# enricobottazzi/zk-fhe

Hardware: AMD Instinct MI355X
Metric: BFV proofs/sec (k=13) (higher is better)
Workload: dtype u32x8 (256-bit Montgomery integers over BN254 Fr/Fq)

## Files before the change

### include/zkfhe.h

```cpp
#ifndef ZKFHE_H
#define ZKFHE_H
#include <stddef.h>
#include <stdint.h>

#ifdef __cplusplus
extern "C" {
#endif

#define ZKFHE_OK 0
#define ZKFHE_EINVAL (-1)
#define ZKFHE_EHIP (-2)
#define ZKFHE_ENOMEM (-3)
#define ZKFHE_ENODEV (-4)

typedef struct zkfhe_ctx zkfhe_ctx;
typedef struct zkfhe_basis zkfhe_basis;

typedef struct { uint64_t l[4]; } zkfhe_fr;
typedef struct { uint64_t l[4]; } zkfhe_fq;
typedef struct { zkfhe_fq x, y; } zkfhe_g1_affine;
typedef struct { zkfhe_fq x, y, zz, zzz; } zkfhe_g1_xyzz;

int zkfhe_ctx_create(int device_id, void *hip_stream, zkfhe_ctx **out);
int zkfhe_ctx_destroy(zkfhe_ctx *ctx);
// ... 166 lines not shown
int zkfhe_srs_table_bits(const zkfhe_srs *srs, int *wide_calls);
int zkfhe_srs_table_info(const zkfhe_srs *srs, int bits[2], uint64_t *bytes, int *narrowed);

typedef struct zkfhe_bfv_pk zkfhe_bfv_pk;
int zkfhe_bfv_keygen(zkfhe_ctx *ctx, const zkfhe_srs *srs, const char *input_json, const zkfhe_bfv_params *params,
                     const zkfhe_bfv_config *config, zkfhe_bfv_pk **out);
int zkfhe_bfv_pk_destroy(zkfhe_ctx *ctx, zkfhe_bfv_pk *pk);
int zkfhe_bfv_pk_release_ctx(zkfhe_ctx *ctx, zkfhe_bfv_pk *pk);
int zkfhe_bfv_pk_info(const zkfhe_bfv_pk *pk, uint8_t vk_digest[32], uint32_t *n_fixed, uint32_t *n_sigma);
int zkfhe_bfv_pk_commitments(const zkfhe_bfv_pk *pk, uint8_t *fixed_out, uint8_t *sigma_out);
int zkfhe_bfv_pk_prefix_cache(const zkfhe_bfv_pk *pk, int capacity, uint64_t *hits, uint64_t *misses, uint64_t *entries);
int zkfhe_bfv_pk_prehash(const zkfhe_bfv_pk *pk, const char *input_json, uint64_t *started, uint64_t *taken, uint64_t *pending);
int zkfhe_bfv_pk_break_points(const zkfhe_bfv_pk *pk, int which, uint32_t *out, uint32_t *count);

int zkfhe_bfv_pk_export_vk(const zkfhe_bfv_pk *pk, uint8_t *out, size_t cap, size_t *len);
int zkfhe_bfv_witness_stream(zkfhe_ctx *ctx, const zkfhe_bfv_pk *pk, const char *input_json, const uint8_t gamma_le[32], uint8_t *cells_out,
                             size_t cap_cells, size_t *n_cells);
int zkfhe_lookup_permute(zkfhe_ctx *ctx, const zkfhe_fr *cols_dev, size_t n_cols, size_t n, uint32_t usable_rows, zkfhe_fr *a_dev,
                         zkfhe_fr *s_dev, int *not_in_table);
int zkfhe_bfv_pk_save(zkfhe_ctx *ctx, const zkfhe_bfv_pk *pk, const char *path);
int zkfhe_bfv_pk_load(zkfhe_ctx *ctx, const zkfhe_srs *srs, const char *path, zkfhe_bfv_pk **out);

int zkfhe_snark_encode(const uint8_t *instances_le, size_t n_instances, const uint8_t *proof, size_t proof_len, uint8_t *out, size_t cap, size_t *len);
int zkfhe_snark_decode(const uint8_t *snark, size_t snark_len, uint8_t *instances_le, size_t *n_instances, uint8_t *proof, size_t *proof_len);

int zkfhe_bfv_verify(const uint8_t *vk_bytes, size_t vk_len, const uint8_t *instances, size_t n_instances, const uint8_t *proof,
                     size_t proof_len, const uint8_t *srs_seed, size_t seed_len, int *accepted, char *err, size_t err_len);
int zkfhe_bfv_verify_g2(const uint8_t *vk_bytes, size_t vk_len, const uint8_t *instances, size_t n_instances, const uint8_t *proof, size_t proof_len,
                        const uint8_t g2[128], const uint8_t s_g2[128], int *accepted, char *err, size_t err_len);

// ... 224 lines not shown
```

### zk-fhe_amd/_abi.py

```python
import ctypes
import os

_HERE = os.path.dirname(os.path.abspath(__file__))
LIB_PATH = os.path.join(_HERE, "libzkfhe_hip.so")
_lib = None

PROF_G1_DECOMPRESS, PROF_MSM_SEGMENTED = 3, 4
PROF_BFV_SAMPLE, PROF_RNS_NTT, PROF_RNS_EPILOGUE = 5, 6, 7
PROF_BFV_TENSOR, PROF_BFV_RELIN, PROF_BFV_EVAL_EPILOGUE, PROF_BFV_ELEMENTWISE = 8, 9, 10, 11
PROF_BFV_SHARE_SUM, PROF_BFV_DECRYPT_COMBINE = 12, 13
PROF_BFV_GALOIS, PROF_BFV_SLOT_NTT = 14, 15
PROF_BFV_HOIST, PROF_BFV_LINEAR = 16, 17
PROF_BFV_BSGS_INNER, PROF_BFV_BSGS_GIANT = 18, 19
PROF_BFV_DOT = 20
PROF_BFV_PCKS_COMBINE, PROF_BFV_REFRESH_COMBINE = 21, 22
PROF_G1_FFT = 23
PROF_BFV_BALLOT = 24
PROF_BFV_RESIDENT = 25
PROF_BFV_KEY_SWITCH_WIDE = 26
PROF_BFV_PACK = 27
BALLOT_COUNTED, BALLOT_SKIPPED, BALLOT_BAD_GROUP, BALLOT_NOT_A_CIPHERTEXT, BALLOT_WRONG_KEY, BALLOT_REJECTED, BALLOT_REPEATED = range(7)
BALLOT_STATUSES = 7
BALLOT_STATUS_NAMES = ("counted", "skipped", "bad_group", "not_a_ciphertext", "wrong_key", "rejected", "repeated")
SRS_BAD_POWERS, SRS_BAD_LAGRANGE, SRS_BAD_GENERATOR = 1, 2, 4
# ... 53 lines not shown
    "zkfhe_comm_record_event": "i:vvv", "zkfhe_g1_add": "i:vvvvn", "zkfhe_g1_mul": "i:vvvvn", "zkfhe_g1_fft": "i:vvii",
    "zkfhe_g1_decompress": "i:vvnvv", "zkfhe_msm_segmented": "i:vvnvvnvnv", "zkfhe_witness_poly_mul_u64": "i:vvvnv",
    "zkfhe_host_poly_mul_u32": "i:ppnpp", "zkfhe_witness_div_mod": "i:vvuvvn", "zkfhe_transcript_create": "i:wV", "zkfhe_transcript_destroy": "-:v",
    "zkfhe_transcript_common_scalar": "i:vs", "zkfhe_transcript_write_scalar": "i:vs", "zkfhe_transcript_common_point": "i:vs",
    "zkfhe_transcript_write_point": "i:vs", "zkfhe_transcript_squeeze": "i:vs", "zkfhe_transcript_bytes": "i:vsnN", "zkfhe_poseidon_permute": "i:s",
    "zkfhe_poseidon_constants": "i:ss", "zkfhe_host_hash_mode": "i:i", "zkfhe_poseidon_hash_many": "i:sNnis", "zkfhe_bfv_build_tables": "i:sBCsiVsn",
    "zkfhe_bfv_tables_free": "-:v", "zkfhe_bfv_auto_config": "i:sBwwwWsn", "zkfhe_bfv_tables_count": "n:vi", "zkfhe_bfv_tables_copy_advice": "i:vp",
    "zkfhe_bfv_tables_copy_fixed": "i:vp", "zkfhe_bfv_tables_copy_instance": "i:vp", "zkfhe_bfv_tables_copy_copies": "i:vp",
    "zkfhe_bfv_tables_copy_break_points": "i:viW", "zkfhe_prover_gate": "i:i", "zkfhe_bfv_mock_check": "i:vspsn",
    "zkfhe_bfv_tables_poke_advice": "i:vwws", "zkfhe_srs_create": "i:vwsnV", "zkfhe_srs_save": "i:vvs", "zkfhe_srs_drop_host_copy": "i:v",
    "zkfhe_srs_load": "i:vsV", "zkfhe_srs_g2": "i:vss", "zkfhe_srs_set_g2": "i:vss", "zkfhe_srs_file_g2": "i:sWss", "zkfhe_chacha20_block": "i:sWs",
    "zkfhe_srs_from_points": "i:vwvvV", "zkfhe_srs_from_monomial": "i:vwvnssV", "zkfhe_srs_load_downsized": "i:vswV", "zkfhe_srs_check": "i:vvsW",
    "zkfhe_srs_create_sharded": "i:vvwsnV", "zkfhe_srs_destroy": "i:vv", "zkfhe_srs_table_bits": "i:vI", "zkfhe_srs_table_info": "i:vIpI",
    "zkfhe_bfv_keygen": "i:vvsBCV", "zkfhe_bfv_pk_destroy": "i:vv", "zkfhe_bfv_pk_release_ctx": "i:vv", "zkfhe_bfv_pk_info": "i:vsWW",
    "zkfhe_bfv_pk_commitments": "i:vss", "zkfhe_bfv_pk_prefix_cache": "i:vippp", "zkfhe_bfv_pk_prehash": "i:vsppp",
    "zkfhe_bfv_pk_break_points": "i:viWW", "zkfhe_bfv_pk_export_vk": "i:vsnN", "zkfhe_bfv_witness_stream": "i:vvssvnN",
    "zkfhe_lookup_permute": "i:vvnnwvvI", "zkfhe_bfv_pk_save": "i:vvs", "zkfhe_bfv_pk_load": "i:vvsV", "zkfhe_snark_encode": "i:snsnsnN",
    "zkfhe_snark_decode": "i:snsNsN", "zkfhe_bfv_verify": "i:snsnsnsnIsn", "zkfhe_bfv_verify_g2": "i:snsnsnssIsn",
    "zkfhe_bfv_verify_batch": "i:vsnnSNSNsnssIsn", "zkfhe_bfv_prove": "i:vvvsssnNsNf", "zkfhe_bfv_prove_words": "i:vvvXssnNsNf",
    "zkfhe_poly_mul_ternary_negacyclic": "i:vvnvnuuvI", "zkfhe_bfv_error_cdt": "i:BpN", "zkfhe_bfv_fhe_keypair": "i:vBsppp",
    "zkfhe_bfv_encrypt": "i:vBppnpsuppppp", "zkfhe_bfv_decrypt": "i:vBpnppp", "zkfhe_bfv_add": "i:vBnppppipp", "zkfhe_bfv_sum": "i:vBnpppp",
    "zkfhe_bfv_add_plain": "i:vBnppnppp", "zkfhe_bfv_mul_plain": "i:vBnppnppp", "zkfhe_bfv_relin_digits": "i:BiN",
    "zkfhe_bfv_relin_keygen": "i:vBpsipp", "zkfhe_bfv_mul": "i:vBnppppppipp", "zkfhe_bfv_noise": "i:vBpnppp", "zkfhe_bfv_dot_max_terms": "i:BiN",
    "zkfhe_bfv_dot": "i:vBnnppnppppipp", "zkfhe_bfv_dot_plain": "i:vBnnppnppp", "zkfhe_bfv_keygen_share": "i:vBssppp",
    "zkfhe_bfv_share_aggregate": "i:vBnnpp", "zkfhe_bfv_relin_share1": "i:vBpssipp", "zkfhe_bfv_relin_share2": "i:vBpsippp",
    "zkfhe_bfv_decrypt_share": "i:vBpnpsuup", "zkfhe_bfv_decrypt_combine": "i:vBnnppp", "zkfhe_bfv_pcks_share": "i:vBpppnpsuupp",
    "zkfhe_bfv_pcks_combine": "i:vBnnppppp", "zkfhe_bfv_refresh_share": "i:vBpsnpsuupp", "zkfhe_bfv_refresh_combine": "i:vBnnsuppppp",
    "zkfhe_bfv_slot_count": "i:BN", "zkfhe_bfv_galois_element": "i:Blip", "zkfhe_bfv_slot_sum_elements": "i:BpN", "zkfhe_bfv_encode_slots": "i:vBnpp",
    "zkfhe_bfv_decode_slots": "i:vBnpp", "zkfhe_bfv_galois_keygen": "i:vBpsuipp", "zkfhe_bfv_apply_galois": "i:vBnppuppipp",
    "zkfhe_bfv_slot_sum": "i:vBnppppipp", "zkfhe_bfv_galois_share": "i:vBpssuipp", "zkfhe_bfv_apply_galois_many": "i:vBnppnpppipp",
    "zkfhe_bfv_linear_transform": "i:vBnppnpppippp", "zkfhe_bfv_linear_transform_bsgs": "i:vBnppnpppnpppippp", "zkfhe_bfv_plan_create": "i:vBnpppipV",
# ... 35 lines not shown
```

### zk-fhe_amd/csrc/fr9.hip.hpp

```cpp
#pragma once
#include "lz29.hip.hpp"

namespace zk {

using Fr9S = Lz<0, 1, 1>;
using Fr9C = Lz<0, 1, 32>;
template <int VV>
using Fr9P = Lz<0, 1, (VV <= 160 ? 2 : 3)>;

ZK_HD Fr9S fr9_load(const Fr &w) { return lz_load(w); }
ZK_HD Fr9S fr9_one() { return lz_load(Fr::one()); }
ZK_HD Fr9C fr9_load32(const Fr &w) {
  Fr9C r;
#pragma unroll
  for (int i = 0; i < 9; ++i) {
    const int bit = 29 * i - 5;
    if (i == 0) {
      r.l[0] = (int)((w.l[0] << 5) & q29::MASK);
    } else {
      const int k = bit >> 5, sh = bit & 31;
      u32 v = w.l[k] >> sh;
      if (sh > 3 && k + 1 < 8) v |= w.l[k + 1] << (32 - sh);
      r.l[i] = (int)(v & q29::MASK);
    }
// ... 50 lines not shown
  Fr9S k;
#pragma unroll
  for (int i = 0; i < 9; ++i) k.l[i] = (int)K[i];
  return fr9_mul(c, k);
}

template <int LO, int HI, int V>
ZK_HD Fr fr9_store(const Lz<LO, HI, V> &a) { return lz_store(a); }

ZK_HD Lz<0, 1, 66> fr9_perm_factor(const Fr9C &v, const Lz<0, 1, 2> &t, const Fr9C &gamma) { return fr9_norm(lz_add(lz_add(v, t), gamma)); }
template <int V>
ZK_HD Lz<0, 1, 3> fr9_perm_step(const Lz<0, 1, V> &acc, const Lz<0, 1, 66> &f) { return lz_widen<0, 1, 3>(fr9_mul(acc, f)); }
ZK_HD Lz<0, 1, 2> fr9_lookup_term(const Fr9S &a, const Fr9S &beta, const Lz<0, 1, 64> &s_gamma) { return fr9_mul(lz_add(a, beta), s_gamma); }
ZK_HD Lz<0, 1, 64> fr9_lookup_sum(const Fr9C &s, const Fr9C &gamma) { return fr9_norm(lz_add(s, gamma)); }

}
```

### zk-fhe_amd/host/keygen.hip

```cpp
#include "prover_internal.hpp"

std::vector<BigInt> GpuPolyMul::mul_u64(const std::vector<uint64_t> &a, const std::vector<uint64_t> &b) {
  const U256 *host = mul_u64_raw(a, b);
  std::vector<BigInt> out(2 * a.size() - 1);
  for (size_t i = 0; i < out.size(); ++i) out[i] = fe::to_bigint(host[i]);
  return out;
}

const U256 *GpuPolyMul::mul_u64_raw(const std::vector<uint64_t> &a, const std::vector<uint64_t> &b) {
  const size_t n = a.size();
  if (ws->polyio.bytes < 2 * n * 8 + 2 * n * 32) throw std::runtime_error("polynomial too long for the prover workspace");
  uint64_t *da = (uint64_t *)ws->polyio.p, *db = da + n;
  Fr *dout = (Fr *)(db + n);
  const U256 *host = ws->host_poly;
  int rc = up(ctx, ws, da, a.data(), n * 8);
  if (!rc) rc = up(ctx, ws, db, b.data(), n * 8);
  if (!rc) rc = zkfhe_witness_poly_mul_u64(ctx, da, db, n, (zkfhe_fr *)dout);
  if (!rc) rc = zkfhe_fr_from_mont(ctx, (const zkfhe_fr *)dout, (zkfhe_fr *)dout, 2 * n - 1);
  if (!rc && ws->host_poly && 2 * n - 1 <= ws->host_poly_len) {
    if (zk_memcpy_async(ctx, ws->host_poly, dout, (2 * n - 1) * 32, hipMemcpyDeviceToHost, ctx->stream) != hipSuccess) rc = ZKFHE_EHIP;
    if (!rc) rc = zkfhe_sync(ctx);
  } else if (!rc) {
    pageable.resize(2 * n - 1);
    host = pageable.data();
// ... 25 lines not shown
    std::vector<U256> l(3 * n, fe::zero());
    const size_t u = cfg.u();
    l[0] = fe::one();
    l[n + u] = fe::one();
    for (size_t i = 0; i < u; ++i) l[2 * n + i] = fe::one();
    CK(upload_canon(ctx, ws->key_l_rows(), l.data(), 3 * n));
    CK(extend_cols(ctx, pk, ws, ws->key_l_rows(), 3, pk->l_ext.fr()));
  }
  {
    const Fr wext = zk_fr_root_of_unity((int)cfg.k + 2);
    Fr shift = mont_u64(COSET_G);
    for (int k1 = 0; k1 < pk->ext_rows; ++k1) {
      zkp::k_powers<<<(unsigned)((n + 255) / 256), 256, 0, ctx->stream>>>(shift, dom->omega, pk->xs_ext.fr() + (size_t)k1 * n, n);
      ZK_LAUNCH_CHECK(ctx);
      shift = shift * wext;
    }
    if (pk->ext_rows == 3) {
      CK(pk->ext3_pw.alloc(ctx, 3 * n * 32));
      Fr gk = mont_u64(COSET_G);
      for (int t = 0; t < 3; ++t) {
        zkp::k_powers<<<(unsigned)((n + 255) / 256), 256, 0, ctx->stream>>>(Fr::one(), fr_inv(gk), pk->ext3_pw.fr() + (size_t)t * n, n);
        ZK_LAUNCH_CHECK(ctx);
        gk = gk * wext;
      }
    }
  }
  return ZKFHE_OK;
}

static U256 vk_digest_of(const zkfhe_bfv_pk *pk) { return vk_digest(pk->cfg, pk->fixed_commit, pk->sigma_commit); }
// ... 117 lines not shown
int zkfhe_bfv_keygen(zkfhe_ctx *ctx, const zkfhe_srs *srs, const char *input_json, const zkfhe_bfv_params *params,
                     const zkfhe_bfv_config *config, zkfhe_bfv_pk **out) {
  ZK_ENTER(ctx);
  ZK_ARG(ctx, srs && input_json && params && config && out);
  try {
    return keygen_impl(ctx, srs, input_json, params_from_c(params), config_from_c(config), config->replay != 0, out);
  } catch (const std::exception &e) {
    return zk_fail_msg(ctx, ZKFHE_EINVAL, e.what());
  }
}

int zkfhe_bfv_pk_destroy(zkfhe_ctx *ctx, zkfhe_bfv_pk *pk) {
  ZK_ENTER(ctx);
  if (!pk) return ZKFHE_OK;
  zkfhe_sync(ctx);
  DevBuf *bufs[] = {&pk->fixed_l, &pk->sigma_l, &pk->fixed_ext, &pk->sigma_ext, &pk->l_ext, &pk->xs_ext, &pk->dpow, &pk->ext3_pw,
                    &pk->lookup_src, &pk->inv_slots, &pk->place_start, &pk->place_len};
  for (DevBuf *b : bufs) b->release();
  for (auto &kv : pk->workspaces) free_workspace(kv.second);
  delete pk;
  return ZKFHE_OK;
}

int zkfhe_bfv_pk_release_ctx(zkfhe_ctx *ctx, zkfhe_bfv_pk *pk) {
  ZK_ENTER(ctx);
  ZK_ARG(ctx, pk != nullptr);
  zkfhe_sync(ctx);
  std::lock_guard<std::mutex> lock(pk->mu);
  auto it = pk->workspaces.find(ctx->uid);
  if (it != pk->workspaces.end()) {
    free_workspace(it->second);
// ... 201 lines not shown
}

int zkfhe_bfv_pk_commitments(const zkfhe_bfv_pk *pk, uint8_t *fixed_out, uint8_t *sigma_out) {
  if (!pk) return ZKFHE_EINVAL;
  for (size_t i = 0; i < pk->fixed_commit.size() && fixed_out; ++i) {
    memcpy(fixed_out + 64 * i, pk->fixed_commit[i].x.l, 32);
    memcpy(fixed_out + 64 * i + 32, pk->fixed_commit[i].y.l, 32);
  }
  for (size_t i = 0; i < pk->sigma_commit.size() && sigma_out; ++i) {
    memcpy(sigma_out + 64 * i, pk->sigma_commit[i].x.l, 32);
    memcpy(sigma_out + 64 * i + 32, pk->sigma_commit[i].y.l, 32);
  }
  return ZKFHE_OK;
}

int zkfhe_bfv_pk_export_vk(const zkfhe_bfv_pk *pk, uint8_t *out, size_t cap, size_t *len) {
  if (!pk || !len) return ZKFHE_EINVAL;
  const size_t nf = pk->fixed_commit.size(), ns = pk->sigma_commit.size();
  const size_t need = 8 + 40 + 32 + 64 * (nf + ns);
  *len = need;
  if (!out || cap < need) return out ? ZKFHE_EINVAL : ZKFHE_OK;
  memcpy(out, "ZKFHEVK2", 8);
  const uint32_t hdr[10] = {pk->cfg.k, pk->cfg.n_gate0, pk->cfg.n_gate1, pk->cfg.n_lookup, pk->cfg.n_rlc, pk->cfg.unusable_rows,
                            pk->cfg.lookup_bits, pk->cfg.transcript, (uint32_t)nf, (uint32_t)ns};
  memcpy(out + 8, hdr, 40);
  memcpy(out + 48, pk->vk_digest.l, 32);
  uint8_t *p = out + 80;
  for (const auto &c : pk->fixed_commit) {
    memcpy(p, c.x.l, 32);
    memcpy(p + 32, c.y.l, 32);
// ... 20 lines not shown
```

### zk-fhe_amd/host/prove.hip

```cpp
#include "prover_internal.hpp"

namespace {

void permute_lookup(const std::vector<U256> &input, size_t u, unsigned table_size, std::vector<U256> &a_perm, std::vector<U256> &s_perm) {
  std::vector<size_t> cnt(table_size, 0);
  for (size_t i = 0; i < u; ++i) {
    const U256 &v = input[i];
    if (v.l[1] | v.l[2] | v.l[3] || v.l[0] >= table_size) throw std::runtime_error("lookup input not in table");
    ++cnt[v.l[0]];
  }
  std::vector<size_t> left(table_size, 1);
  left[0] = u - (table_size - 1);
  a_perm.assign(u, fe::zero());
  s_perm.assign(u, fe::zero());
  std::vector<size_t> holes;
  size_t pos = 0;
  for (unsigned v = 0; v < table_size; ++v)
    for (size_t k = 0; k < cnt[v]; ++k, ++pos) {
      a_perm[pos] = fe::from_u64(v);
      if (k == 0) {
        if (!left[v]) throw std::runtime_error("lookup input not in table");
        --left[v];
        s_perm[pos] = fe::from_u64(v);
      } else {
// ... 846 lines not shown
    }
    return ZKFHE_OK;
  }
  zkp::QArgs quotient_args(const zkp::QGroup *groups_dev, int q_rows) const {
    zkp::QArgs qa;
    qa.adv = ws->adv_ext.fr();
    qa.fix = pk->fixed_ext.fr();
    qa.sig = pk->sigma_ext.fr();
    qa.pz = ws->pz_ext.fr();
    qa.lz = ws->lz_ext.fr();
    qa.la = ws->la_ext.fr();
    qa.ls = ws->ls_ext.fr();
    qa.inst = ws->inst_ext.fr();
    qa.lext = pk->l_ext.fr();
    qa.xs = pk->xs_ext.fr();
    qa.beta_delta = beta_delta_dev;
    qa.groups = groups_dev;
    qa.partials = ws->quotient_partials();
    qa.y = y;
    qa.beta = beta;
    qa.gamma = gamma;
    qa.gamma_rlc = mont(gamma_rlc);
    qa.log_n = k;
    qa.u = (unsigned)u;
    qa.n_gate = cfg.n_gate();
    qa.n_rlc = cfg.n_rlc;
    qa.adv_rlc0 = cfg.adv_rlc0();
    qa.fix_qrlc0 = cfg.fix_qrlc0();
    qa.fix_const = cfg.fix_const();
    qa.fix_table = cfg.fix_table();
    qa.adv_lookup0 = cfg.adv_lookup0();
    qa.n_lookup = cfg.n_lookup;
    qa.n_advice = cfg.n_advice();
    qa.n_perm = cfg.n_perm();
    qa.chunk = cfg.chunk();
    qa.n_chunks = cfg.n_chunks();
    qa.rows = (unsigned)q_rows;
    return qa;
  }
  int launch_quotient(zkp::QArgs &qa, size_t pt0, size_t count, size_t G, const Fr *ypow_dev, const Fr *zinv_dev) {
    qa.pt0 = pt0;
    qa.pt_count = count;
    const unsigned blocks = (unsigned)((count + 255) / 256);
    if (G) {
      zkp::k_quotient_partials<<<dim3(blocks, (unsigned)G), 256, 0, ctx->stream>>>(qa);
      ZK_LAUNCH_CHECK(ctx);
    }
    zkp::k_quotient_combine<<<blocks, 256, 0, ctx->stream>>>(ws->quotient_partials(), ypow_dev, (unsigned)G, zinv_dev, k, qa.rows, pt0, count, ws->h_ext.fr());
    ZK_LAUNCH_CHECK(ctx);
    return ZKFHE_OK;
  }
  int quotient(std::vector<AffinePoint> &h_commit) {
    const int q_rows = pk->ext_rows;
    const Fr wext = zk_fr_root_of_unity((int)k + 2);
    if (W_sh == 1) {
      CK(extend_cols(ctx, pk, ws, ws->all_l.fr(), ws->n_all, ws->all_ext.fr()));
    } else {
      const size_t ecol = n * (size_t)q_rows;
      auto ext_range = [&](const View &l, const View &e, size_t lo, size_t hi) -> int {
        if (hi <= lo) return ZKFHE_OK;
        return extend_cols(ctx, pk, ws, l.fr() + lo * n, hi - lo, e.fr() + lo * ecol);
      };
      const size_t a_lo = std::min<size_t>(c_lo * cfg.chunk(), cfg.n_advice()), a_hi = std::min<size_t>(c_hi * cfg.chunk(), cfg.n_advice());
      CK(ext_range(ws->adv_l, ws->adv_ext, a_lo, a_hi));
      const size_t l_lo = a_lo > cfg.adv_lookup0() ? std::min<size_t>(a_lo - cfg.adv_lookup0(), cfg.n_lookup) : 0;
      const size_t l_hi = a_hi > cfg.adv_lookup0() ? std::min<size_t>(a_hi - cfg.adv_lookup0(), cfg.n_lookup) : 0;
      CK(ext_range(ws->la_l, ws->la_ext, l_lo, l_hi));
      CK(ext_range(ws->ls_l, ws->ls_ext, l_lo, l_hi));
      CK(ext_range(ws->lz_l, ws->lz_ext, l_lo, l_hi));
// ... 12 lines not shown
          ++j;
          continue;
        }
        size_t len = 0;
        while (j + len < first + count && len < max_group && owned(j + len)) ++len;
        groups.push_back(zkp::QGroup{type, (int)j, (int)len, 0});
        e += len * expr_per_unit;
        last_e.push_back(e - 1);
        j += len;
      }
    };
    run(zkp::QG_GATE, 0, cfg.n_gate(), 8, 1, [&](size_t j) { return owns_col(j); });
    run(zkp::QG_RLC, 0, cfg.n_rlc, cfg.n_rlc ? cfg.n_rlc : 1, 1, [&](size_t j) { return owns_col(cfg.adv_rlc0() + j); });
    run(zkp::QG_PERM_FIRST, 0, 1, 1, 1, [&](size_t) { return owns_chunk(0); });
    run(zkp::QG_PERM_LAST, 0, 1, 1, 1, [&](size_t) { return owns_chunk(nch - 1); });
    run(zkp::QG_PERM_C, 1, nch - 1, 32, 1, [&](size_t j) { return owns_chunk(j); });
    run(zkp::QG_PERM_D, 0, nch, 4, 1, [&](size_t j) { return owns_chunk(j); });
    run(zkp::QG_LOOKUP, 0, cfg.n_lookup, 3, 5, [&](size_t i) { return owns_col(cfg.adv_lookup0() + i); });
    const size_t E = e, G = groups.size();
    if (G > 96 || G * n * (size_t)q_rows * 32 > ws->cap(wsl::QUOTIENT_PARTIALS)) return zk_fail_msg(ctx, ZKFHE_EINVAL, "too many quotient groups for the workspace");
    std::vector<Fr> ypow(G);
    for (size_t g = 0; g < G; ++g) ypow[g] = zk::zk_fr_to_29(fr_pow(y, E - 1 - last_e[g]));
    if (groups.empty()) groups.push_back(zkp::QGroup{});
    if (ypow.empty()) ypow.push_back(Fr::zero());
    STAGE(groups_dev, zkp::QGroup, ws, groups.data(), groups.size() * sizeof(zkp::QGroup));
    STAGE(ypow_dev, Fr, ws, ypow.data(), ypow.size() * 32);
    const Fr gn = fr_pow(mont_u64(COSET_G), n), i4 = fr_pow(wext, n);
    Fr zinv[4], cur = gn;
    for (int t = 0; t < 4; ++t) {
      zinv[t] = zk::zk_fr_to_29(fr_inv(cur - Fr::one()));
      cur = cur * i4;
    }
    STAGE(zinv_dev, Fr, ws, zinv, 4 * 32);
// ... 498 lines not shown
```

### zk-fhe_amd/host/prover_internal.hpp

```cpp
#pragma once
#include <chrono>
#include <ctime>
#include <cstdio>
#include <cstring>
#include <map>
#include <atomic>
#include <mutex>
#include <thread>
#include <stdexcept>

#include "../../include/zkfhe.h"
#include "bfv_circuit.hpp"
#include "bfv_phase0_fast.hpp"
#include "gpu_witness.hip.hpp"
#include "prover_kernels.hip.hpp"
#include "shplonk.hpp"
#include "transcript.hpp"
#include "prefix_cache.hpp"
#include "vk.hpp"

using namespace zkhost;
using zk::Fr;
using zk::G1Affine;

// ... 128 lines not shown
  zkfhe_ctx *ctx;
  Workspace *ws;
  GpuPolyMul(zkfhe_ctx *c, Workspace *w) : ctx(c), ws(w) {}
  std::vector<BigInt> mul_u64(const std::vector<uint64_t> &a, const std::vector<uint64_t> &b) override;
  const U256 *mul_u64_raw(const std::vector<uint64_t> &a, const std::vector<uint64_t> &b) override;

 private:
  std::vector<U256> pageable;
};


struct zkfhe_bfv_pk {
  CircuitConfig cfg;
  BfvParams prm;
  DevBuf fixed_l, sigma_l, fixed_ext, sigma_ext, l_ext, xs_ext, dpow, ext3_pw;
  std::vector<AffinePoint> fixed_commit, sigma_commit;
  U256 vk_digest;
  size_t gate1_cells = 0, n_lookup_cells = 0, n_inv_slots = 0;
  int ext_rows = 3;
  DevBuf lookup_src, inv_slots, place_start, place_len;
  std::map<uint64_t, Workspace *> workspaces;
  std::mutex mu;
  PrefixCache prefix;
  PreHash prehash;
};
```

### zk-fhe_amd/host/prover_kernels.hip.hpp

```cpp
#pragma once
#include "../csrc/ctx.hpp"
#include "../csrc/fr9.hip.hpp"
#include "chain_jobs.hpp"

namespace zkp {

using zk::Fr;

__device__ __forceinline__ void powers_body(Fr start, Fr base, Fr *__restrict__ out, size_t n, unsigned blk, unsigned nblk) {
  for (size_t i = blk * (size_t)blockDim.x + threadIdx.x; i < n; i += (size_t)nblk * blockDim.x) {
    Fr r = start, b = base;
    for (size_t e = i; e; e >>= 1) {
      if (e & 1) r = r * b;
      b = zk::fp_sqr<zk::FrP>(b);
    }
    out[i] = r;
  }
}
static __global__ void __launch_bounds__(256) k_powers(Fr start, Fr base, Fr *__restrict__ out, size_t n) { powers_body(start, base, out, n, blockIdx.x, gridDim.x); }

__device__ __forceinline__ unsigned long long rotr64(unsigned long long x, int n) { return (x >> n) | (x << (64 - n)); }
__device__ __forceinline__ Fr rng_draw(const unsigned long long seed[4], unsigned long long ctr) {
  typedef unsigned long long u64;
  const u64 IV[8] = {0x6a09e667f3bcc908ULL, 0xbb67ae8584caa73bULL, 0x3c6ef372fe94f82bULL, 0xa54ff53a5f1d36f1ULL,
// ... 319 lines not shown
}
static __global__ void __launch_bounds__(1024) k_chunk_carry_both(Fr *__restrict__ total, unsigned n_carry, unsigned n_ones, int *__restrict__ closes) {
  if (blockIdx.x == 0) chunk_carry_body(total, n_carry, 0, closes);
  else chunk_carry_body(total + n_carry, n_ones, 1, closes + 1);
}
static __global__ void __launch_bounds__(256) k_scale_rows(Fr *__restrict__ z, const Fr *__restrict__ carry, size_t n, unsigned rows, unsigned n_cols) {
  const size_t total = (size_t)n_cols * rows;
  for (size_t g = blockIdx.x * (size_t)blockDim.x + threadIdx.x; g < total; g += (size_t)gridDim.x * blockDim.x) {
    const unsigned col = (unsigned)(g / rows);
    const unsigned i = (unsigned)(g - (size_t)col * rows);
    Fr *p = z + (size_t)col * n + i;
    *p = *p * carry[col];
  }
}

enum { QG_GATE = 0, QG_RLC = 1, QG_PERM_HEAD = 2, QG_PERM_C = 3, QG_PERM_D = 4, QG_LOOKUP = 5, QG_PERM_FIRST = 6, QG_PERM_LAST = 7 };
struct QGroup {
  int type, first, count, pad;
};
struct QArgs {
  const Fr *adv, *fix, *sig, *pz, *lz, *la, *ls, *inst, *lext, *xs;
  const Fr *beta_delta;
  const QGroup *groups;
  Fr *partials;
  Fr y, beta, gamma, gamma_rlc;
  unsigned log_n, u, n_gate, n_rlc, adv_rlc0, fix_qrlc0, fix_const, fix_table, adv_lookup0, n_lookup, n_advice, n_perm, chunk, n_chunks;
  unsigned rows;
  size_t pt0, pt_count;
};

static __global__ void __launch_bounds__(256) k_quotient_partials(QArgs a) {
  const size_t n = (size_t)1 << a.log_n, ne = n * a.rows;
  const size_t p = a.pt0 + blockIdx.x * (size_t)blockDim.x + threadIdx.x;
  if (p >= a.pt0 + a.pt_count || p >= ne) return;
  const QGroup g = a.groups[blockIdx.y];
  const size_t row0 = p & ~(n - 1);
  const size_t k2 = p & (n - 1);
  auto at = [&](const Fr *base, unsigned col, unsigned rot) -> Fr { return base[(size_t)col * ne + row0 + ((k2 + rot) & (n - 1))]; };
  auto ld = [&](const Fr *base, unsigned col, unsigned rot) { return zk::fr9_load(at(base, col, rot)); };
  auto ld32 = [&](const Fr *base, unsigned col, unsigned rot) { return zk::fr9_load32(at(base, col, rot)); };
  const zk::Fr9C y = zk::fr9_load32(a.y);
  zk::Lz<0, 1, 3> acc = zk::lz_widen<0, 1, 3>(zk::lz_zero());
  auto horner = [&](const zk::Fr9C &u, const auto &v) { acc = zk::lz_widen<0, 1, 3>(zk::fr9_mul2(acc, y, u, v)); };
  switch (g.type) {
// ... 16 lines not shown
    case QG_PERM_HEAD: {
      const Fr zm = at(a.pz, a.n_chunks - 1, 0);
      acc = zk::lz_widen<0, 1, 3>(zk::fr9_mul(zk::fr9_load32(a.lext[p]), zk::lz_sub(zk::fr9_one(), ld(a.pz, 0, 0))));
      horner(zk::fr9_load32(a.lext[ne + p]), zk::lz_sub(zk::fr9_mul(zk::fr9_load(zm), zk::fr9_load32(zm)), zk::fr9_load(zm)));
      break;
    }
    case QG_PERM_FIRST:
      acc = zk::lz_widen<0, 1, 3>(zk::fr9_mul(zk::fr9_load32(a.lext[p]), zk::lz_sub(zk::fr9_one(), ld(a.pz, 0, 0))));
      break;
    case QG_PERM_LAST: {
      const Fr zm = at(a.pz, a.n_chunks - 1, 0);
      acc = zk::lz_widen<0, 1, 3>(zk::fr9_mul(zk::fr9_load32(a.lext[ne + p]), zk::lz_sub(zk::fr9_mul(zk::fr9_load(zm), zk::fr9_load32(zm)), zk::fr9_load(zm))));
      break;
    }
    case QG_PERM_C: {
      const zk::Fr9C l0 = zk::fr9_load32(a.lext[p]);
      for (int j = g.first; j < g.first + g.count; ++j) horner(l0, zk::lz_sub(ld(a.pz, j, 0), ld(a.pz, j - 1, a.u)));
      break;
    }
    case QG_PERM_D: {
      const zk::Fr9C lact = zk::fr9_load32(a.lext[2 * ne + p]), gamma = zk::fr9_load32(a.gamma);
      const zk::Lz<0, 1, 2> beta = zk::fr9_cc(zk::fr9_load32(a.beta)), x = zk::fr9_cc(zk::fr9_load32(a.xs[p]));
      for (int j = g.first; j < g.first + g.count; ++j) {
        zk::Lz<0, 1, 3> left = zk::lz_widen<0, 1, 3>(ld(a.pz, j, 1)), right = zk::lz_widen<0, 1, 3>(ld(a.pz, j, 0));
        for (unsigned c = j * a.chunk; c < (j + 1) * a.chunk && c < a.n_perm; ++c) {
          const zk::Fr9C v = zk::fr9_load32(c < a.n_advice ? at(a.adv, c, 0) : (c == a.n_advice ? at(a.fix, a.fix_const, 0) : a.inst[p]));
          left = zk::fr9_perm_step(left, zk::fr9_perm_factor(v, zk::fr9_mul(ld(a.sig, c, 0), beta), gamma));
          right = zk::fr9_perm_step(right, zk::fr9_perm_factor(v, zk::fr9_mul(zk::fr9_load(a.beta_delta[c]), x), gamma));
        }
        horner(lact, zk::lz_sub(left, right));
      }
      break;
    }
    case QG_LOOKUP: {
      const zk::Fr9C l0 = zk::fr9_load32(a.lext[p]), ll = zk::fr9_load32(a.lext[ne + p]), lact = zk::fr9_load32(a.lext[2 * ne + p]);
      const zk::Fr9C gamma = zk::fr9_load32(a.gamma);
      const zk::Fr9S beta = zk::fr9_load(a.beta), one = zk::fr9_one();
      const zk::Lz<0, 1, 64> s_gamma = zk::fr9_lookup_sum(ld32(a.fix, a.fix_table, 0), gamma);
      for (int i = g.first; i < g.first + g.count; ++i) {
        const Fr z0 = at(a.lz, i, 0), ap = at(a.la, i, 0), sp = at(a.ls, i, 0);
        const auto d = zk::lz_sub(zk::fr9_load(ap), zk::fr9_load(sp));
        horner(l0, zk::lz_sub(one, zk::fr9_load(z0)));
        horner(ll, zk::lz_sub(zk::fr9_mul(zk::fr9_load(z0), zk::fr9_load32(z0)), zk::fr9_load(z0)));
        horner(lact, zk::fr9_mul2(ld32(a.lz, i, 1), zk::fr9_lookup_term(zk::fr9_load(ap), beta, zk::fr9_lookup_sum(zk::fr9_load32(sp), gamma)), zk::fr9_load32(z0),
                                  zk::lz_neg(zk::fr9_lookup_term(ld(a.adv, a.adv_lookup0 + i, 0), beta, s_gamma))));
        horner(l0, d);
        horner(lact, zk::fr9_mul(zk::lz_sub(zk::fr9_load32(ap), ld32(a.la, i, (unsigned)(n - 1))), d));
      }
      break;
    }
  }
  a.partials[(size_t)blockIdx.y * ne + p] = zk::fr9_store(acc);
}

static __global__ void __launch_bounds__(256) k_quotient_combine(const Fr *__restrict__ partials, const Fr *__restrict__ ypow, unsigned n_groups,
                                                          const Fr *__restrict__ zinv, unsigned log_n, unsigned rows, size_t pt0, size_t pt_count, Fr *__restrict__ h_ext) {
  const size_t n = (size_t)1 << log_n, ne = n * rows;
  const size_t p = pt0 + blockIdx.x * (size_t)blockDim.x + threadIdx.x;
  if (p >= pt0 + pt_count || p >= ne) return;
  zk::F29 acc;
#pragma unroll
  for (int l = 0; l < 9; ++l) acc.l[l] = 0;
  unsigned g = 0;
// ... 190 lines not shown
```

### zk-fhe_amd/prover.py

```python
import ctypes
import os

import numpy as np

from ._abi import ALLGATHER_FN, _U64P, ZkfheError, _BfvWordsC, load_library
from .hostonly import Instances, _g2_bytes, _g2_tuple, seed32


class Comm:

    def __init__(self, ctx, rank, world, unique_id=None, all_gather=None):
        self.ctx, self.rank, self.world = ctx, rank, world
        self.h = ctypes.c_void_p()
        if world > 1 and unique_id is None and all_gather is None:
            raise ValueError("Comm(world > 1) needs a transport: unique_id= (RCCL) or all_gather= (a host all-gather callable)")
        if unique_id is None:
            def cb(_user, send, nbytes, recv):
                try:
                    parts = all_gather(ctypes.string_at(send, nbytes))
                    data = b"".join(parts)
                    if len(data) != nbytes * world:
                        return 1
                    ctypes.memmove(recv, data, len(data))
                    return 0
# ... 242 lines not shown
    def prehash(self, input_json_text=None):
        s, t, p = ctypes.c_uint64(), ctypes.c_uint64(), ctypes.c_uint64()
        text = None if input_json_text is None else (input_json_text if isinstance(input_json_text, bytes) else input_json_text.encode())
        rc = self.ctx.lib.zkfhe_bfv_pk_prehash(self.h, text, ctypes.byref(s), ctypes.byref(t), ctypes.byref(p))
        if rc != 0:
            raise ZkfheError("zkfhe_bfv_pk_prehash: too many announced proofs are pending (%d)" % rc)
        return {"started": s.value, "taken": t.value, "pending": p.value}

    def export_vk(self):
        lib = self.ctx.lib
        n = ctypes.c_size_t()
        lib.zkfhe_bfv_pk_export_vk(self.h, None, 0, ctypes.byref(n))
        buf = ctypes.create_string_buffer(n.value)
        self.ctx._check(lib.zkfhe_bfv_pk_export_vk(self.h, buf, n.value, ctypes.byref(n)))
        return buf.raw

    def destroy(self):
        if self.h:
            self.ctx.lib.zkfhe_bfv_pk_destroy(self.ctx.h, self.h)
            self.h = None


def bfv_verify_batch(ctx, vk_bytes, items, srs_seed=b"zkfhe-unsafe-srs", g2=None, s_g2=None):
    lib = load_library()
    items = list(items)
    n = len(items)
    enc_inst = lambda v: v.raw if isinstance(v, Instances) else b"".join(int(x).to_bytes(32, "little") for x in v)
    insts = [enc_inst(i) for i, _ in items]
    proofs = [bytes(p) for _, p in items]
    keep = insts + proofs
# ... 20 lines not shown
```

Before: 278.9.

## Precompute delta·x table and restructure quotient groups as y-power dot sums

At keygen, for domains up to 65536, a table of delta^c·x over the extended domain is precomputed and stored in the proving key. The permutation factors are rescaled by 1/beta so each step needs one multiply less. The sequential Horner accumulations in the PERM_C, PERM_D and LOOKUP quotient groups become sums weighted by precomputed y powers, accumulated lazily, followed by one multiply by the Lagrange term. This shortens the serial multiply dependency chains and removes per-column beta·delta·x multiplies. In exchange it adds device memory for the table, a host-side inverse of beta, and a new error path when beta is zero.

After: 275.8. 0.989x the previous value.

```diff
diff --git a/include/zkfhe.h b/include/zkfhe.h
--- a/include/zkfhe.h
+++ b/include/zkfhe.h
@@ -204,6 +204,7 @@
 int zkfhe_bfv_pk_break_points(const zkfhe_bfv_pk *pk, int which, uint32_t *out, uint32_t *count);
 
 int zkfhe_bfv_pk_export_vk(const zkfhe_bfv_pk *pk, uint8_t *out, size_t cap, size_t *len);
+int zkfhe_bfv_pk_dx_table(zkfhe_ctx *ctx, const zkfhe_bfv_pk *pk, uint8_t *out, size_t cap, size_t *len);
 int zkfhe_bfv_witness_stream(zkfhe_ctx *ctx, const zkfhe_bfv_pk *pk, const char *input_json, const uint8_t gamma_le[32], uint8_t *cells_out,
                              size_t cap_cells, size_t *n_cells);
 int zkfhe_lookup_permute(zkfhe_ctx *ctx, const zkfhe_fr *cols_dev, size_t n_cols, size_t n, uint32_t usable_rows, zkfhe_fr *a_dev,
diff --git a/zk-fhe_amd/_abi.py b/zk-fhe_amd/_abi.py
--- a/zk-fhe_amd/_abi.py
+++ b/zk-fhe_amd/_abi.py
@@ -91,7 +91,7 @@
     "zkfhe_srs_create_sharded": "i:vvwsnV", "zkfhe_srs_destroy": "i:vv", "zkfhe_srs_table_bits": "i:vI", "zkfhe_srs_table_info": "i:vIpI",
     "zkfhe_bfv_keygen": "i:vvsBCV", "zkfhe_bfv_pk_destroy": "i:vv", "zkfhe_bfv_pk_release_ctx": "i:vv", "zkfhe_bfv_pk_info": "i:vsWW",
     "zkfhe_bfv_pk_commitments": "i:vss", "zkfhe_bfv_pk_prefix_cache": "i:vippp", "zkfhe_bfv_pk_prehash": "i:vsppp",
-    "zkfhe_bfv_pk_break_points": "i:viWW", "zkfhe_bfv_pk_export_vk": "i:vsnN", "zkfhe_bfv_witness_stream": "i:vvssvnN",
+    "zkfhe_bfv_pk_break_points": "i:viWW", "zkfhe_bfv_pk_export_vk": "i:vsnN", "zkfhe_bfv_pk_dx_table": "i:vvsnN", "zkfhe_bfv_witness_stream": "i:vvssvnN",
     "zkfhe_lookup_permute": "i:vvnnwvvI", "zkfhe_bfv_pk_save": "i:vvs", "zkfhe_bfv_pk_load": "i:vvsV", "zkfhe_snark_encode": "i:snsnsnN",
     "zkfhe_snark_decode": "i:snsNsN", "zkfhe_bfv_verify": "i:snsnsnsnIsn", "zkfhe_bfv_verify_g2": "i:snsnsnssIsn",
     "zkfhe_bfv_verify_batch": "i:vsnnSNSNsnssIsn", "zkfhe_bfv_prove": "i:vvvsssnNsNf", "zkfhe_bfv_prove_words": "i:vvvXssnNsNf",
diff --git a/zk-fhe_amd/csrc/fr9.hip.hpp b/zk-fhe_amd/csrc/fr9.hip.hpp
--- a/zk-fhe_amd/csrc/fr9.hip.hpp
+++ b/zk-fhe_amd/csrc/fr9.hip.hpp
@@ -88,4 +88,30 @@
 ZK_HD Lz<0, 1, 2> fr9_lookup_term(const Fr9S &a, const Fr9S &beta, const Lz<0, 1, 64> &s_gamma) { return fr9_mul(lz_add(a, beta), s_gamma); }
 ZK_HD Lz<0, 1, 64> fr9_lookup_sum(const Fr9C &s, const Fr9C &gamma) { return fr9_norm(lz_add(s, gamma)); }
 
+using Fr9K = Fr9S;
+using Fr9Sum = LzW;
+ZK_HD Fr9K fr9_const(const Fr &w29 ) { return lz_load(w29); }
+ZK_HD Fr9Sum fr9_sum_zero() {
+  Fr9Sum s;
+#pragma unroll
+  for (int i = 0; i < 9; ++i) s.l[i] = 0;
+  return s;
 }
+template <int LO, int HI, int V>
+ZK_HD Fr9Sum fr9_sum_add(const Fr9Sum &s, const Fr9K &c, const Lz<LO, HI, V> &x) {
+  static_assert(V <= 160, "sum term: the product comes back below 2 r in magnitude, the sum below 4 r: inside the weak reduction's 16 r");
+  return lz_weak(lz_add(s, fr9_mul(c, x)));
+}
+template <int L0, int H0, int V0, int L1, int H1, int V1>
+ZK_HD Fr9Sum fr9_sum_add2(const Fr9Sum &s, const Fr9K &c0, const Lz<L0, H0, V0> &x0, const Fr9K &c1, const Lz<L1, H1, V1> &x1) {
+  static_assert(V0 + V1 <= 160, "sum terms: the two products come back below 2 r in magnitude, the sum below 4 r");
+  return lz_weak(lz_add(s, fr9_mul2(c0, x0, c1, x1)));
+}
+ZK_HD Lz<0, 1, 3> fr9_dot3(const Fr9C &l0, const Fr9Sum &s0, const Fr9C &l1, const Fr9Sum &s1, const Fr9C &l2, const Fr9Sum &s2) {
+  return mont29_c<fr29_mod, u64, u32, Lz<0, 1, 3>>(l0, s0, l1, s1, l2, s2);
+}
+ZK_HD Lz<0, 1, 66> fr9_perm_factor_pp(const Lz<0, 1, 2> &v, const Lz<0, 1, 2> &t, const Fr9C &gamma) {
+  return lz_widen<0, 1, 66>(fr9_norm(lz_add(lz_add(v, t), gamma)));
+}
+
+}
diff --git a/zk-fhe_amd/host/keygen.hip b/zk-fhe_amd/host/keygen.hip
--- a/zk-fhe_amd/host/keygen.hip
+++ b/zk-fhe_amd/host/keygen.hip
@@ -63,6 +63,11 @@
       zkp::k_powers<<<(unsigned)((n + 255) / 256), 256, 0, ctx->stream>>>(shift, dom->omega, pk->xs_ext.fr() + (size_t)k1 * n, n);
       ZK_LAUNCH_CHECK(ctx);
       shift = shift * wext;
+    }
+    if (n <= 65536) {
+      CK(pk->dx_ext.alloc(ctx, cells * R * 32));
+      zkp::k_column_multiples<<<dim3((unsigned)((R * n + 255) / 256), cfg.n_perm()), 256, 0, ctx->stream>>>(pk->dpow.fr(), pk->xs_ext.fr(), R * n, pk->dx_ext.fr());
+      ZK_LAUNCH_CHECK(ctx);
     }
     if (pk->ext_rows == 3) {
       CK(pk->ext3_pw.alloc(ctx, 3 * n * 32));
@@ -210,7 +215,7 @@
   ZK_ENTER(ctx);
   if (!pk) return ZKFHE_OK;
   zkfhe_sync(ctx);
-  DevBuf *bufs[] = {&pk->fixed_l, &pk->sigma_l, &pk->fixed_ext, &pk->sigma_ext, &pk->l_ext, &pk->xs_ext, &pk->dpow, &pk->ext3_pw,
+  DevBuf *bufs[] = {&pk->fixed_l, &pk->sigma_l, &pk->fixed_ext, &pk->sigma_ext, &pk->l_ext, &pk->xs_ext, &pk->dpow, &pk->ext3_pw, &pk->dx_ext,
                     &pk->lookup_src, &pk->inv_slots, &pk->place_start, &pk->place_len};
   for (DevBuf *b : bufs) b->release();
   for (auto &kv : pk->workspaces) free_workspace(kv.second);
@@ -442,6 +447,16 @@
   return ZKFHE_OK;
 }
 
+int zkfhe_bfv_pk_dx_table(zkfhe_ctx *ctx, const zkfhe_bfv_pk *pk, uint8_t *out, size_t cap, size_t *len) {
+  ZK_ENTER(ctx);
+  ZK_ARG(ctx, pk && len);
+  const size_t need = pk->dx_ext.p ? pk->dx_ext.bytes : 0;
+  *len = need;
+  if (!out || !need) return ZKFHE_OK;
+  ZK_ARG(ctx, cap >= need);
+  return zkfhe_download(ctx, out, pk->dx_ext.p, need);
+}
+
 int zkfhe_bfv_pk_export_vk(const zkfhe_bfv_pk *pk, uint8_t *out, size_t cap, size_t *len) {
   if (!pk || !len) return ZKFHE_EINVAL;
   const size_t nf = pk->fixed_commit.size(), ns = pk->sigma_commit.size();
diff --git a/zk-fhe_amd/host/prove.hip b/zk-fhe_amd/host/prove.hip
--- a/zk-fhe_amd/host/prove.hip
+++ b/zk-fhe_amd/host/prove.hip
@@ -884,13 +884,10 @@
     qa.inst = ws->inst_ext.fr();
     qa.lext = pk->l_ext.fr();
     qa.xs = pk->xs_ext.fr();
-    qa.beta_delta = beta_delta_dev;
+    qa.dx = pk->dx_ext.p ? pk->dx_ext.fr() : nullptr;
+    qa.dpow = pk->dpow.fr();
     qa.groups = groups_dev;
     qa.partials = ws->quotient_partials();
-    qa.y = y;
-    qa.beta = beta;
-    qa.gamma = gamma;
-    qa.gamma_rlc = mont(gamma_rlc);
     qa.log_n = k;
     qa.u = (unsigned)u;
     qa.n_gate = cfg.n_gate();
@@ -906,6 +903,7 @@
     qa.chunk = cfg.chunk();
     qa.n_chunks = cfg.n_chunks();
     qa.rows = (unsigned)q_rows;
+    zkp::quotient_challenges(qa, y, beta, gamma, mont(gamma_rlc));
     return qa;
   }
   int launch_quotient(zkp::QArgs &qa, size_t pt0, size_t count, size_t G, const Fr *ypow_dev, const Fr *zinv_dev) {
@@ -923,6 +921,7 @@
   int quotient(std::vector<AffinePoint> &h_commit) {
     const int q_rows = pk->ext_rows;
     const Fr wext = zk_fr_root_of_unity((int)k + 2);
+    if (beta.is_zero()) return zk_fail_msg(ctx, ZKFHE_EINVAL, "the challenge beta is zero: the quotient divides the permutation factors by it");
     if (W_sh == 1) {
       CK(extend_cols(ctx, pk, ws, ws->all_l.fr(), ws->n_all, ws->all_ext.fr()));
     } else {
@@ -965,9 +964,9 @@
     run(zkp::QG_RLC, 0, cfg.n_rlc, cfg.n_rlc ? cfg.n_rlc : 1, 1, [&](size_t j) { return owns_col(cfg.adv_rlc0() + j); });
     run(zkp::QG_PERM_FIRST, 0, 1, 1, 1, [&](size_t) { return owns_chunk(0); });
     run(zkp::QG_PERM_LAST, 0, 1, 1, 1, [&](size_t) { return owns_chunk(nch - 1); });
-    run(zkp::QG_PERM_C, 1, nch - 1, 32, 1, [&](size_t j) { return owns_chunk(j); });
-    run(zkp::QG_PERM_D, 0, nch, 4, 1, [&](size_t j) { return owns_chunk(j); });
-    run(zkp::QG_LOOKUP, 0, cfg.n_lookup, 3, 5, [&](size_t i) { return owns_col(cfg.adv_lookup0() + i); });
+    run(zkp::QG_PERM_C, 1, nch - 1, zkp::QG_MAX_PERM_C, 1, [&](size_t j) { return owns_chunk(j); });
+    run(zkp::QG_PERM_D, 0, nch, zkp::QG_MAX_PERM_D, 1, [&](size_t j) { return owns_chunk(j); });
+    run(zkp::QG_LOOKUP, 0, cfg.n_lookup, zkp::QG_MAX_LOOKUP, 5, [&](size_t i) { return owns_col(cfg.adv_lookup0() + i); });
     const size_t E = e, G = groups.size();
     if (G > 96 || G * n * (size_t)q_rows * 32 > ws->cap(wsl::QUOTIENT_PARTIALS)) return zk_fail_msg(ctx, ZKFHE_EINVAL, "too many quotient groups for the workspace");
     std::vector<Fr> ypow(G);
diff --git a/zk-fhe_amd/host/prover_internal.hpp b/zk-fhe_amd/host/prover_internal.hpp
--- a/zk-fhe_amd/host/prover_internal.hpp
+++ b/zk-fhe_amd/host/prover_internal.hpp
@@ -166,6 +166,7 @@
   CircuitConfig cfg;
   BfvParams prm;
   DevBuf fixed_l, sigma_l, fixed_ext, sigma_ext, l_ext, xs_ext, dpow, ext3_pw;
+  DevBuf dx_ext;
   std::vector<AffinePoint> fixed_commit, sigma_commit;
   U256 vk_digest;
   size_t gate1_cells = 0, n_lookup_cells = 0, n_inv_slots = 0;
diff --git a/zk-fhe_amd/host/prover_kernels.hip.hpp b/zk-fhe_amd/host/prover_kernels.hip.hpp
--- a/zk-fhe_amd/host/prover_kernels.hip.hpp
+++ b/zk-fhe_amd/host/prover_kernels.hip.hpp
@@ -357,20 +357,52 @@
   }
 }
 
+static __global__ void __launch_bounds__(256) k_column_multiples(const Fr *__restrict__ mult, const Fr *__restrict__ row, size_t len, Fr *__restrict__ out) {
+  const size_t i = blockIdx.x * (size_t)blockDim.x + threadIdx.x;
+  if (i < len) out[(size_t)blockIdx.y * len + i] = mult[blockIdx.y] * row[i];
+}
 enum { QG_GATE = 0, QG_RLC = 1, QG_PERM_HEAD = 2, QG_PERM_C = 3, QG_PERM_D = 4, QG_LOOKUP = 5, QG_PERM_FIRST = 6, QG_PERM_LAST = 7 };
 struct QGroup {
   int type, first, count, pad;
 };
 struct QArgs {
   const Fr *adv, *fix, *sig, *pz, *lz, *la, *ls, *inst, *lext, *xs;
-  const Fr *beta_delta;
+  const Fr *dx;
+  const Fr *dpow;
   const QGroup *groups;
   Fr *partials;
   Fr y, beta, gamma, gamma_rlc;
+  Fr gamma_b, beta_inv_cc;
+  Fr ypow[32], yb[4], yb_last[4];
   unsigned log_n, u, n_gate, n_rlc, adv_rlc0, fix_qrlc0, fix_const, fix_table, adv_lookup0, n_lookup, n_advice, n_perm, chunk, n_chunks;
   unsigned rows;
   size_t pt0, pt_count;
 };
+enum { QG_MAX_PERM_C = 32, QG_MAX_PERM_D = 4, QG_MAX_LOOKUP = 3 };
+inline void quotient_challenges(QArgs &qa, const Fr &y, const Fr &beta, const Fr &gamma, const Fr &gamma_rlc) {
+  qa.y = y;
+  qa.beta = beta;
+  qa.gamma = gamma;
+  qa.gamma_rlc = gamma_rlc;
+  const Fr beta_inv = zk::fp_inv<zk::FrP>(beta);
+  qa.gamma_b = gamma * beta_inv;
+  qa.beta_inv_cc = zk::zk_fr_to_29(zk::zk_fr_to_29(beta_inv));
+  const unsigned m_last = qa.n_perm - (qa.n_chunks - 1) * qa.chunk;
+  Fr b_full = Fr::one(), b_last = Fr::one();
+  for (unsigned i = 0; i < qa.chunk; ++i) {
+    b_full = b_full * beta;
+    if (i < m_last) b_last = b_last * beta;
+  }
+  Fr yp = Fr::one();
+  for (int i = 0; i < 32; ++i) {
+    qa.ypow[i] = zk::zk_fr_to_29(yp);
+    if (i < 4) {
+      qa.yb[i] = zk::zk_fr_to_29(yp * b_full);
+      qa.yb_last[i] = zk::zk_fr_to_29(yp * b_last);
+    }
+    yp = yp * y;
+  }
+}
 
 static __global__ void __launch_bounds__(256) k_quotient_partials(QArgs a) {
   const size_t n = (size_t)1 << a.log_n, ne = n * a.rows;
@@ -417,39 +449,56 @@
       break;
     }
     case QG_PERM_C: {
-      const zk::Fr9C l0 = zk::fr9_load32(a.lext[p]);
-      for (int j = g.first; j < g.first + g.count; ++j) horner(l0, zk::lz_sub(ld(a.pz, j, 0), ld(a.pz, j - 1, a.u)));
+      const int last = g.first + g.count - 1;
+      auto diff = [&](int j) { return zk::lz_sub(ld(a.pz, j, 0), ld(a.pz, j - 1, a.u)); };
+      zk::Fr9Sum s = zk::fr9_sum_zero();
+      int j = g.first;
+      for (; j < last; j += 2) s = zk::fr9_sum_add2(s, zk::fr9_const(a.ypow[last - j]), diff(j), zk::fr9_const(a.ypow[last - j - 1]), diff(j + 1));
+      if (j == last) s = zk::fr9_sum_add(s, zk::fr9_const(a.ypow[0]), diff(j));
+      acc = zk::lz_widen<0, 1, 3>(zk::fr9_mul(zk::fr9_load32(a.lext[p]), s));
       break;
     }
     case QG_PERM_D: {
-      const zk::Fr9C lact = zk::fr9_load32(a.lext[2 * ne + p]), gamma = zk::fr9_load32(a.gamma);
-      const zk::Lz<0, 1, 2> beta = zk::fr9_cc(zk::fr9_load32(a.beta)), x = zk::fr9_cc(zk::fr9_load32(a.xs[p]));
-      for (int j = g.first; j < g.first + g.count; ++j) {
+      const zk::Fr9C gamma = zk::fr9_load32(a.gamma_b);
+      const zk::Fr9K beta_inv = zk::fr9_const(a.beta_inv_cc);
+      zk::Lz<0, 1, 2> x = zk::lz_widen<0, 1, 2>(zk::lz_zero());
+      if (!a.dx) x = zk::fr9_cc(zk::fr9_load32(a.xs[p]));
+      const int last = g.first + g.count - 1;
+      auto diff = [&](int j) {
         zk::Lz<0, 1, 3> left = zk::lz_widen<0, 1, 3>(ld(a.pz, j, 1)), right = zk::lz_widen<0, 1, 3>(ld(a.pz, j, 0));
         for (unsigned c = j * a.chunk; c < (j + 1) * a.chunk && c < a.n_perm; ++c) {
-          const zk::Fr9C v = zk::fr9_load32(c < a.n_advice ? at(a.adv, c, 0) : (c == a.n_advice ? at(a.fix, a.fix_const, 0) : a.inst[p]));
-          left = zk::fr9_perm_step(left, zk::fr9_perm_factor(v, zk::fr9_mul(ld(a.sig, c, 0), beta), gamma));
-          right = zk::fr9_perm_step(right, zk::fr9_perm_factor(v, zk::fr9_mul(zk::fr9_load(a.beta_delta[c]), x), gamma));
+          const zk::Lz<0, 1, 2> v = zk::fr9_mul(zk::fr9_load(c < a.n_advice ? at(a.adv, c, 0) : (c == a.n_advice ? at(a.fix, a.fix_const, 0) : a.inst[p])), beta_inv);
+          left = zk::fr9_perm_step(left, zk::fr9_perm_factor(ld32(a.sig, c, 0), v, gamma));
+          if (a.dx) right = zk::fr9_perm_step(right, zk::fr9_perm_factor(ld32(a.dx, c, 0), v, gamma));
+          else right = zk::fr9_perm_step(right, zk::fr9_perm_factor_pp(v, zk::fr9_mul(zk::fr9_load(a.dpow[c]), x), gamma));
         }
-        horner(lact, zk::lz_sub(left, right));
-      }
+        return zk::lz_sub(left, right);
+      };
+      auto coef = [&](int j) { return zk::fr9_const(j + 1 == (int)a.n_chunks ? a.yb_last[last - j] : a.yb[last - j]); };
+      zk::Fr9Sum s = zk::fr9_sum_zero();
+      int j = g.first;
+      for (; j < last; j += 2) s = zk::fr9_sum_add2(s, coef(j), diff(j), coef(j + 1), diff(j + 1));
+      if (j == last) s = zk::fr9_sum_add(s, coef(j), diff(j));
+      acc = zk::lz_widen<0, 1, 3>(zk::fr9_mul(zk::fr9_load32(a.lext[2 * ne + p]), s));
       break;
     }
     case QG_LOOKUP: {
-      const zk::Fr9C l0 = zk::fr9_load32(a.lext[p]), ll = zk::fr9_load32(a.lext[ne + p]), lact = zk::fr9_load32(a.lext[2 * ne + p]);
       const zk::Fr9C gamma = zk::fr9_load32(a.gamma);
       const zk::Fr9S beta = zk::fr9_load(a.beta), one = zk::fr9_one();
       const zk::Lz<0, 1, 64> s_gamma = zk::fr9_lookup_sum(ld32(a.fix, a.fix_table, 0), gamma);
+      zk::Fr9Sum s0 = zk::fr9_sum_zero(), s1 = zk::fr9_sum_zero(), s2 = zk::fr9_sum_zero();
       for (int i = g.first; i < g.first + g.count; ++i) {
+        const Fr *c = a.ypow + 5 * (g.first + g.count - 1 - i);
         const Fr z0 = at(a.lz, i, 0), ap = at(a.la, i, 0), sp = at(a.ls, i, 0);
         const auto d = zk::lz_sub(zk::fr9_load(ap), zk::fr9_load(sp));
-        horner(l0, zk::lz_sub(one, zk::fr9_load(z0)));
-        horner(ll, zk::lz_sub(zk::fr9_mul(zk::fr9_load(z0), zk::fr9_load32(z0)), zk::fr9_load(z0)));
-        horner(lact, zk::fr9_mul2(ld32(a.lz, i, 1), zk::fr9_lookup_term(zk::fr9_load(ap), beta, zk::fr9_lookup_sum(zk::fr9_load32(sp), gamma)), zk::fr9_load32(z0),
-                                  zk::lz_neg(zk::fr9_lookup_term(ld(a.adv, a.adv_lookup0 + i, 0), beta, s_gamma))));
-        horner(l0, d);
-        horner(lact, zk::fr9_mul(zk::lz_sub(zk::fr9_load32(ap), ld32(a.la, i, (unsigned)(n - 1))), d));
+        s0 = zk::fr9_sum_add2(s0, zk::fr9_const(c[4]), zk::lz_sub(one, zk::fr9_load(z0)), zk::fr9_const(c[1]), d);
+        s1 = zk::fr9_sum_add(s1, zk::fr9_const(c[3]), zk::lz_sub(zk::fr9_mul(zk::fr9_load(z0), zk::fr9_load32(z0)), zk::fr9_load(z0)));
+        s2 = zk::fr9_sum_add2(s2, zk::fr9_const(c[2]),
+                              zk::fr9_mul2(ld32(a.lz, i, 1), zk::fr9_lookup_term(zk::fr9_load(ap), beta, zk::fr9_lookup_sum(zk::fr9_load32(sp), gamma)), zk::fr9_load32(z0),
+                                           zk::lz_neg(zk::fr9_lookup_term(ld(a.adv, a.adv_lookup0 + i, 0), beta, s_gamma))),
+                              zk::fr9_const(c[0]), zk::fr9_mul(zk::lz_sub(zk::fr9_load32(ap), ld32(a.la, i, (unsigned)(n - 1))), d));
       }
+      acc = zk::fr9_dot3(zk::fr9_load32(a.lext[p]), s0, zk::fr9_load32(a.lext[ne + p]), s1, zk::fr9_load32(a.lext[2 * ne + p]), s2);
       break;
     }
   }
diff --git a/zk-fhe_amd/prover.py b/zk-fhe_amd/prover.py
--- a/zk-fhe_amd/prover.py
+++ b/zk-fhe_amd/prover.py
@@ -280,6 +280,14 @@
         buf = ctypes.create_string_buffer(n.value)
         self.ctx._check(lib.zkfhe_bfv_pk_export_vk(self.h, buf, n.value, ctypes.byref(n)))
         return buf.raw
+
+    def dx_table(self):
+        lib = self.ctx.lib
+        n = ctypes.c_size_t()
+        self.ctx._check(lib.zkfhe_bfv_pk_dx_table(self.ctx.h, self.h, None, 0, ctypes.byref(n)))
+        buf = ctypes.create_string_buffer(max(1, n.value))
+        self.ctx._check(lib.zkfhe_bfv_pk_dx_table(self.ctx.h, self.h, buf, n.value, ctypes.byref(n)))
+        return buf.raw[: n.value]
 
     def destroy(self):
         if self.h:
```
